# NVIDIA/spark-rapids

Measured on AMD Instinct MI355X. Metric: NDS power-run fact rows/s from on-disk parquet (speedup vs CPU backend in config), higher is better.
Workload: dtype decimal(7,2)+fp64+string-keys

## Files before the change

### native/hipdf/include/hipdf.h

```cpp
#ifndef HIPDF_H
#define HIPDF_H

#include <hip/hip_runtime.h>
#include <stddef.h>
#include <stdint.h>

#ifdef __cplusplus
#define HIPDF_STATIC_ASSERT(cond, msg) static_assert(cond, msg)
extern "C" {
#else
#define HIPDF_STATIC_ASSERT(cond, msg) _Static_assert(cond, msg)
#endif

typedef enum {
  HIPDF_U8 = 0,
  HIPDF_I8 = 1,
  HIPDF_I16 = 2,
  HIPDF_I32 = 3,
  HIPDF_I64 = 4,
  HIPDF_F32 = 5,
  HIPDF_F64 = 6,
} HipdfType;

typedef struct {
// ... 520 lines not shown
                           const void* stop, const void* bvalid,
                           const void* step, const void* svalid,
                           void* out_len, void* vout, void* err, int64_t n,
                           hipStream_t stream);
void hipdf_sequence_fill(int t, const void* offs, const void* start,
                         const void* stop, const void* step, int64_t n,
                         void* out, int64_t total, hipStream_t stream);
void hipdf_array_join_sizes(const void* offsets, const void* rvalid,
                            const void* eoffs, const void* cvalid, int dlen,
                            int rlen, int64_t n, void* contrib, int64_t total,
                            hipStream_t stream);
void hipdf_array_join_rows(const void* offsets, const void* scanned, int dlen,
                           int64_t n, void* out_len, hipStream_t stream);
void hipdf_array_join_write(const void* offsets, const void* rvalid,
                            const void* eoffs, const void* bytes,
                            const void* cvalid, const void* delim, int dlen,
                            const void* repl, int rlen, const void* scanned,
                            const void* out_off, int64_t n, void* out,
                            int64_t total, hipStream_t stream);

int64_t hipdf_pq_plain_pieces(const void* chunk, int64_t nbytes,
                              int64_t num_values, int max_def, int phys_width,
                              int64_t* out, int64_t max_out);

typedef struct {
  const void* src;
  int64_t nbytes;
  int32_t phys_width;
  int32_t dst_width;
  void* dst;
  int64_t num_values;
  int32_t group;
  int32_t max_def;
} HipdfScanChunk;
HIPDF_STATIC_ASSERT(sizeof(HipdfScanChunk) == 48, "packed as <qqiiqqii");

typedef struct HipdfScanReader HipdfScanReader;
HipdfScanReader* hipdf_scan_open(int n_threads, int n_streams,
                                 int64_t piece_bytes);
int64_t hipdf_scan_submit(HipdfScanReader* r, const HipdfScanChunk* chunks,
                          int64_t n_chunks, int n_groups,
                          hipStream_t consumer);
int hipdf_scan_wait_group(HipdfScanReader* r, int64_t ticket, int group,
                          hipStream_t consumer);
void hipdf_scan_cancel(HipdfScanReader* r, int64_t ticket);
void hipdf_scan_close(HipdfScanReader* r);

int hipdf_pool_init(double fraction, size_t bytes);
int hipdf_pool_active(void);
typedef int (*hipdf_failure_cb)(size_t needed, int retry);
void hipdf_pool_set_failure_cb(hipdf_failure_cb cb);
size_t hipdf_pool_used(void);
size_t hipdf_pool_reserved(void);
size_t hipdf_pool_high_watermark(void);
size_t hipdf_pool_overflow(void);
void* hipdf_pool_alloc(size_t n);
void hipdf_pool_free(void* p);
void* hipdf_torch_malloc(size_t size, int device, hipStream_t stream);
void hipdf_torch_free(void* ptr, size_t size, int device,
                      hipStream_t stream);
int hipdf_pool_selftest(void);

#ifdef __cplusplus
}
#endif
#undef HIPDF_STATIC_ASSERT

#endif
// ... 1 lines not shown
```

### native/hipdf/kernels/pq_pieces.h

```cpp
#ifndef HIPDF_PQ_PIECES_H
#define HIPDF_PQ_PIECES_H

#include <stdint.h>

namespace pq_pieces {

constexpr int64_t kErrTruncated = -1;
constexpr int64_t kErrDictionary = -2;
constexpr int64_t kErrEncoding = -3;
constexpr int64_t kErrCompressed = -4;
constexpr int64_t kErrWidth = -5;
constexpr int64_t kErrNulls = -6;
constexpr int64_t kErrNested = -7;
constexpr int64_t kErrMalformed = -8;
constexpr int64_t kErrCapacity = -9;
constexpr int64_t kErrCount = -10;

struct Cursor {
  const uint8_t* p;
  int64_t pos;
  int64_t end;
  bool ok;

  int byte() {
// ... 92 lines not shown
      return 0;
    }
    return last;
  }
};

inline void skip_struct(Cursor& c, int depth) {
  if (depth > 8) {
    c.ok = false;
    return;
  }
  Fields f(c);
  int t;
  while (f.next(&t)) skip_value(c, t, depth);
}

inline bool rle_all_valid(const uint8_t* lv, int64_t nb, int64_t n,
                          int max_def) {
  Cursor c{lv, 0, nb, true};
  int64_t seen = 0;
  while (seen < n) {
    uint64_t h = c.varint();
    if (!c.ok) return false;
    if (h & 1) return false;
    uint64_t count = h >> 1;
    int v = c.byte();
    if (!c.ok || v != max_def || count == 0) return false;
    if (count > (uint64_t)(n - seen)) count = (uint64_t)(n - seen);
    seen += (int64_t)count;
  }
  return true;
}

inline int64_t walk(const uint8_t* chunk, int64_t nbytes, int64_t num_values,
                    int max_def, int phys_width, int64_t* out,
                    int64_t max_out) {
  if (phys_width != 4 && phys_width != 8) return kErrWidth;
  if (nbytes < 0 || num_values < 0 || max_def < 0 || max_def > 127)
    return kErrMalformed;
  Cursor c{chunk, 0, nbytes, true};
  int64_t decoded = 0, npages = 0;
  while (decoded < num_values && c.pos < nbytes) {
    int64_t type = -1, usize = -1, csize = -1;
    int64_t n = -1, enc = -1, nulls = 0, def_len = 0, rep_len = 0;
    bool v2 = false, have_dp = false, v2_compressed = true;
    Fields f(c);
    int t;
    int fid;
    while ((fid = f.next(&t)) != 0) {
      if (fid == 1 && t == CT_I32) {
        type = c.zigzag();
      } else if (fid == 2 && t == CT_I32) {
        usize = c.zigzag();
      } else if (fid == 3 && t == CT_I32) {
        csize = c.zigzag();
      } else if (fid == 5 && t == CT_STRUCT) {
        have_dp = true;
        Fields g(c);
        int t2, f2;
        while ((f2 = g.next(&t2)) != 0) {
          if (f2 == 1 && t2 == CT_I32)
            n = c.zigzag();
          else if (f2 == 2 && t2 == CT_I32)
            enc = c.zigzag();
          else
            skip_value(c, t2, 1);
        }
      } else if (fid == 7 && t == CT_STRUCT) {
        return kErrDictionary;
      } else if (fid == 8 && t == CT_STRUCT) {
        have_dp = v2 = true;
        Fields g(c);
        int t2, f2;
        while ((f2 = g.next(&t2)) != 0) {
          if (f2 == 1 && t2 == CT_I32)
            n = c.zigzag();
          else if (f2 == 2 && t2 == CT_I32)
            nulls = c.zigzag();
          else if (f2 == 4 && t2 == CT_I32)
            enc = c.zigzag();
          else if (f2 == 5 && t2 == CT_I32)
            def_len = c.zigzag();
          else if (f2 == 6 && t2 == CT_I32)
            rep_len = c.zigzag();
          else if (f2 == 7 && (t2 == CT_TRUE || t2 == CT_FALSE))
            v2_compressed = t2 == CT_TRUE;
          else
            skip_value(c, t2, 1);
        }
      } else {
        skip_value(c, t, 0);
      }
      if (!c.ok) return kErrTruncated;
    }
    if (!c.ok) return kErrTruncated;
    if (type == 2) return kErrDictionary;
    if ((type != 0 && type != 3) || !have_dp || (type == 3) != v2)
      return kErrMalformed;
    if (usize < 0 || csize < 0 || n < 0) return kErrMalformed;
    if (csize > nbytes - c.pos) return kErrTruncated;
    if (enc != 0) return kErrEncoding;
    if (csize != usize) return kErrCompressed;
    const int64_t page = c.pos;
    int64_t vpos = 0;
    if (!v2) {
      if (max_def > 0) {
        if (csize < 4) return kErrTruncated;
        uint32_t len = (uint32_t)chunk[page] | (uint32_t)chunk[page + 1] << 8 |
                       (uint32_t)chunk[page + 2] << 16 |
                       (uint32_t)chunk[page + 3] << 24;
        if ((int64_t)len > csize - 4) return kErrTruncated;
        if (!rle_all_valid(chunk + page + 4, (int64_t)len, n, max_def))
          return kErrNulls;
        vpos = 4 + (int64_t)len;
      }
    } else {
      if (rep_len != 0) return kErrNested;
      if (def_len < 0 || def_len > csize) return kErrMalformed;
      if (max_def > 0) {
        if (nulls != 0) return kErrNulls;
        if (!rle_all_valid(chunk + page, def_len, n, max_def))
          return kErrNulls;
      } else if (def_len != 0) {
        return kErrMalformed;
      }
      (void)v2_compressed;
      vpos = def_len;
    }
    if (csize - vpos != n * (int64_t)phys_width) return kErrCompressed;
    if (n > num_values - decoded) return kErrCount;
    if (npages >= max_out) return kErrCapacity;
    out[3 * npages] = page + vpos;
    out[3 * npages + 1] = n * (int64_t)phys_width;
    out[3 * npages + 2] = n;
    ++npages;
    decoded += n;
    c.pos = page + csize;
  }
  if (decoded != num_values) return decoded < num_values ? kErrTruncated
                                                         : kErrCount;
  return npages;
}

}

#endif
```

### native/hipdf/scan_reader.hip

```cpp
#include <hip/hip_runtime.h>

#include <algorithm>
#include <condition_variable>
#include <deque>
#include <memory>
#include <mutex>
#include <thread>
#include <vector>

#include "hipdf.h"
#include "pq_pieces.h"

namespace {

__global__ void k_widen_i32_i64(const int32_t* __restrict__ in,
                                int64_t* __restrict__ out, int64_t n) {
  int64_t i = (int64_t)blockIdx.x * blockDim.x + threadIdx.x;
  int64_t stride = (int64_t)gridDim.x * blockDim.x;
  for (; i < n; i += stride) out[i] = (int64_t)in[i];
}

struct Piece {
  const uint8_t* src;
  uint8_t* dst;
  int64_t nbytes;
  int32_t widen;
  int32_t group;
};

struct Group {
  int64_t total = 0;
  int64_t enqueued = 0;
  int open_workers = 0;
  std::vector<hipEvent_t> events;
  bool waited = false;
};

struct Submit {
  int64_t ticket = 0;
  std::vector<Piece> pieces;
  size_t next = 0;
  std::vector<Group> groups;
  hipEvent_t start = nullptr;
  int in_flight = 0;
  bool cancelled = false;
  int error = 0;
  std::vector<char> stream_used;

  bool group_ready(int g) const {
    const Group& gr = groups[(size_t)g];
    return gr.enqueued == gr.total && gr.open_workers == 0;
  }
  bool exhausted() const { return cancelled || next >= pieces.size(); }
};

}

struct HipdfScanReader {
  int device = 0;
  int64_t piece_bytes = 0;
  std::vector<std::thread> threads;
  std::vector<hipStream_t> streams;
  std::vector<hipStream_t> owned_streams;
  std::vector<void*> scratch;
  std::mutex mu;
  std::condition_variable work_cv;
  std::condition_variable done_cv;
  std::deque<std::shared_ptr<Submit>> queue;
  std::vector<std::shared_ptr<Submit>> live;
  int64_t next_ticket = 1;
  bool stop = false;

  std::shared_ptr<Submit> find(int64_t ticket) {
    for (auto& s : live)
      if (s->ticket == ticket) return s;
    return nullptr;
  }

  void leave_group(Submit& s, int g, int w) {
    hipEvent_t ev = nullptr;
    hipError_t e = hipEventCreateWithFlags(&ev, hipEventDisableTiming);
    if (e == hipSuccess) e = hipEventRecord(ev, streams[(size_t)w]);
    std::lock_guard<std::mutex> lk(mu);
    if (e != hipSuccess && !s.error) s.error = (int)e;
    if (ev) s.groups[(size_t)g].events.push_back(ev);
    --s.groups[(size_t)g].open_workers;
    done_cv.notify_all();
  }

  void worker(int w) {
    (void)hipSetDevice(device);
    std::shared_ptr<Submit> cur;
    int cur_group = -1;
    for (;;) {
      std::shared_ptr<Submit> s;
      size_t idx = 0;
      {
        std::unique_lock<std::mutex> lk(mu);
        for (;;) {
          while (!queue.empty() && queue.front()->exhausted())
            queue.pop_front();
          if (stop || !queue.empty()) break;
          if (cur) break;
          work_cv.wait(lk);
        }
        if (!stop && !queue.empty()) {
          s = queue.front();
          idx = s->next++;
          int g = s->pieces[idx].group;
          if (s != cur || g != cur_group) ++s->groups[(size_t)g].open_workers;
          ++s->in_flight;
        }
      }
      if (cur && (!s || s != cur || s->pieces[idx].group != cur_group)) {
        leave_group(*cur, cur_group, w);
        cur.reset();
        cur_group = -1;
      }
      if (!s) {
        std::lock_guard<std::mutex> lk(mu);
        if (stop) return;
        continue;
      }
      const Piece& p = s->pieces[idx];
      hipStream_t st = streams[(size_t)w];
      hipError_t e = hipSuccess;
      if (!s->stream_used[(size_t)w]) {
        e = hipStreamWaitEvent(st, s->start, 0);
        s->stream_used[(size_t)w] = 1;
      }
      if (e == hipSuccess) {
        if (!p.widen) {
          e = hipMemcpyAsync(p.dst, p.src, (size_t)p.nbytes,
                             hipMemcpyHostToDevice, st);
        } else {
          e = hipMemcpyAsync(scratch[(size_t)w], p.src, (size_t)p.nbytes,
                             hipMemcpyHostToDevice, st);
          if (e == hipSuccess) {
            int64_t n = p.nbytes / 4;
            int blocks = (int)std::min<int64_t>((n + 255) / 256, 4096);
            hipLaunchKernelGGL(k_widen_i32_i64, dim3((unsigned)blocks),
                               dim3(256), 0, st,
                               (const int32_t*)scratch[(size_t)w],
                               (int64_t*)p.dst, n);
            e = hipGetLastError();
          }
        }
      }
      cur = s;
      cur_group = p.group;
      {
        std::lock_guard<std::mutex> lk(mu);
        if (e != hipSuccess && !s->error) s->error = (int)e;
        ++s->groups[(size_t)p.group].enqueued;
        --s->in_flight;
        done_cv.notify_all();
      }
    }
  }
};

extern "C" {

int64_t hipdf_pq_plain_pieces(const void* chunk, int64_t nbytes,
                              int64_t num_values, int max_def, int phys_width,
                              int64_t* out, int64_t max_out) {
  return pq_pieces::walk((const uint8_t*)chunk, nbytes, num_values, max_def,
                         phys_width, out, max_out);
}

HipdfScanReader* hipdf_scan_open(int n_threads, int n_streams,
                                 int64_t piece_bytes) {
  n_threads = std::max(1, std::min(n_threads, 8));
  n_streams = std::max(1, std::min(n_streams, n_threads));
  piece_bytes = std::max<int64_t>(piece_bytes, 64) / 8 * 8;
  auto* r = new HipdfScanReader();
  r->piece_bytes = piece_bytes;
  if (hipGetDevice(&r->device) != hipSuccess) {
    delete r;
    return nullptr;
  }
  bool ok = true;
  for (int i = 0; i < n_streams && ok; ++i) {
    hipStream_t st = nullptr;
    ok = hipStreamCreateWithFlags(&st, hipStreamNonBlocking) == hipSuccess;
    if (ok) r->owned_streams.push_back(st);
  }
  for (int w = 0; w < n_threads && ok; ++w) {
    void* p = nullptr;
    ok = hipMalloc(&p, (size_t)piece_bytes) == hipSuccess;
    if (ok) r->scratch.push_back(p);
  }
  if (!ok) {
    for (void* p : r->scratch) (void)hipFree(p);
    for (hipStream_t st : r->owned_streams) (void)hipStreamDestroy(st);
    delete r;
    return nullptr;
  }
  for (int w = 0; w < n_threads; ++w)
    r->streams.push_back(r->owned_streams[(size_t)(w % n_streams)]);
  for (int w = 0; w < n_threads; ++w)
    r->threads.emplace_back([r, w] { r->worker(w); });
  return r;
}

int64_t hipdf_scan_submit(HipdfScanReader* r, const HipdfScanChunk* chunks,
                          int64_t n_chunks, int n_groups,
                          hipStream_t consumer) {
  if (!r || n_chunks < 0 || n_groups < 0) return -100;
  auto s = std::make_shared<Submit>();
  s->groups.resize((size_t)n_groups);
  s->stream_used.assign(r->threads.size(), 0);
  std::vector<int64_t> pages;
  for (int64_t i = 0; i < n_chunks; ++i) {
    const HipdfScanChunk& c = chunks[i];
    if (c.group < 0 || c.group >= n_groups) return -100;
    bool widen = c.phys_width == 4 && c.dst_width == 8;
    if (!widen && c.dst_width != c.phys_width) return pq_pieces::kErrWidth;
    if (pages.empty()) pages.resize(3 * 256);
    int64_t np;
    for (;;) {
      np = pq_pieces::walk((const uint8_t*)c.src, c.nbytes, c.num_values,
                           c.max_def, c.phys_width, pages.data(),
                           (int64_t)pages.size() / 3);
      if (np != pq_pieces::kErrCapacity || pages.size() >= (3u << 22)) break;
      pages.resize(pages.size() * 4);
    }
    if (np < 0) return np;
    int64_t row = 0;
    for (int64_t k = 0; k < np; ++k) {
      int64_t off = pages[(size_t)(3 * k)], nb = pages[(size_t)(3 * k + 1)];
      for (int64_t done = 0; done < nb; done += r->piece_bytes) {
        int64_t take = std::min(r->piece_bytes, nb - done);
        Piece p;
        p.src = (const uint8_t*)c.src + off + done;
        p.dst = (uint8_t*)c.dst +
                (row + done / c.phys_width) * (int64_t)c.dst_width;
        p.nbytes = take;
        p.widen = widen ? 1 : 0;
        p.group = c.group;
        s->pieces.push_back(p);
      }
      row += pages[(size_t)(3 * k + 2)];
    }
  }
  std::stable_sort(s->pieces.begin(), s->pieces.end(),
                   [](const Piece& a, const Piece& b) {
                     return a.group < b.group;
                   });
  for (const Piece& p : s->pieces) ++s->groups[(size_t)p.group].total;
  if (hipEventCreateWithFlags(&s->start, hipEventDisableTiming) != hipSuccess)
    return -101;
  if (hipEventRecord(s->start, consumer) != hipSuccess) {
// ... 23 lines not shown
  for (hipEvent_t ev : g.events)
    if (hipStreamWaitEvent(consumer, ev, 0) != hipSuccess) return -102;
  g.waited = true;
  return 0;
}

void hipdf_scan_cancel(HipdfScanReader* r, int64_t ticket) {
  if (!r) return;
  std::shared_ptr<Submit> s;
  bool drain = false;
  {
    std::unique_lock<std::mutex> lk(r->mu);
    s = r->find(ticket);
    if (!s) return;
    s->cancelled = true;
    r->work_cv.notify_all();
    r->done_cv.notify_all();
    r->done_cv.wait(lk, [&] {
      if (s->in_flight) return false;
      for (const Group& g : s->groups)
        if (g.open_workers) return false;
      return true;
    });
    for (const Group& g : s->groups)
      if (!g.waited && g.enqueued) drain = true;
    r->live.erase(std::find(r->live.begin(), r->live.end(), s));
  }
  if (drain)
    for (size_t w = 0; w < s->stream_used.size(); ++w)
      if (s->stream_used[w]) (void)hipStreamSynchronize(r->streams[w]);
  for (Group& g : s->groups)
    for (hipEvent_t ev : g.events) (void)hipEventDestroy(ev);
  (void)hipEventDestroy(s->start);
}

void hipdf_scan_close(HipdfScanReader* r) {
  if (!r) return;
  std::vector<int64_t> tickets;
  {
    std::lock_guard<std::mutex> lk(r->mu);
    for (auto& s : r->live) tickets.push_back(s->ticket);
  }
  for (int64_t t : tickets) hipdf_scan_cancel(r, t);
  {
    std::lock_guard<std::mutex> lk(r->mu);
    r->stop = true;
    r->work_cv.notify_all();
    r->done_cv.notify_all();
  }
  for (std::thread& t : r->threads) t.join();
  for (hipStream_t st : r->owned_streams) {
    (void)hipStreamSynchronize(st);
    (void)hipStreamDestroy(st);
  }
  for (void* p : r->scratch) (void)hipFree(p);
  delete r;
}

}
```

### spark_rapids_amd/api.py

```python
from __future__ import annotations

from typing import Dict, Iterable, List, Optional, Sequence, Union

import numpy as np

from .column import Column, ColumnBatch, Field, Schema
from .config import RapidsConf, CONCURRENT_GPU_TASKS
from .expr.aggregates import AggExpr
from .expr.expressions import Expression, col as _col
from .memory.semaphore import GpuSemaphore
from .plan import logical as L
from .plan.overrides import plan_physical
from .types import DType, INT32, TypeId


class MemTable:

    def __init__(self, batches: List[ColumnBatch], schema: Schema,
                 replicated: bool = False):
        self.batches = batches
        self.schema = schema
        self.replicated = replicated

    def partitions(self) -> Iterable[ColumnBatch]:
# ... 449 lines not shown
                    pending, nbytes = [], 0
                pending.append(b)
                nbytes += b.nbytes
            if pending:
                merged.append(pending[0] if len(pending) == 1
                              else _ops.concat_batches(pending))
            batches = merged
        return DataFrame(self, L.Scan(MemTable(batches, schema, replicated),
                                      schema, label))

    def register(self, name: str, df: DataFrame):
        self.catalog[name] = df

    def table(self, name: str) -> DataFrame:
        return self.catalog[name]

    def sql(self, query: str) -> DataFrame:
        from .sql.parser import parse_sql

        return parse_sql(self, query)

    def read_parquet(self, path: str, columns=None,
                     replicated: bool = False) -> DataFrame:
        import torch

        from .config import PARQUET_MT_THREADS, PARQUET_READER_TYPE
        from .io.parquet import ParquetTable

        reader = str(self.conf.get(PARQUET_READER_TYPE)).upper()
        if reader == "AUTO":
            reader = "GPU_DECODE" if (torch.cuda.is_available()
                                      and self.conf.sql_enabled) else "CPU"
        from .config import (BATCH_SIZE_BYTES, PARQUET_STREAM_SCAN,
                             PARQUET_STREAM_SCAN_FILES)

        src = ParquetTable(path, columns=columns, reader=reader,
                           prefetch_threads=self.conf.get(PARQUET_MT_THREADS),
                           replicated=replicated,
                           chunk_bytes=self.conf.get(BATCH_SIZE_BYTES),
                           stream_scan=self.conf.get(PARQUET_STREAM_SCAN),
                           stream_files=self.conf.get(
                               PARQUET_STREAM_SCAN_FILES))
        return DataFrame(self, L.Scan(src, src.schema, f"parquet:{path}"))

    def write_parquet(self, df: DataFrame, path: str,
                      compression: str = "snappy",
                      gpu_encode: bool = False):
        if gpu_encode:
            from . import ops as _ops
            from .io.parquet_write import write_parquet_gpu

            exec_ = df.physical_plan()
            sem = GpuSemaphore.get()
            with sem.held():
                root = exec_
                while type(root).__name__ == "DeviceTransferExec":
                    root = root.children[0]
                batches = list(root.execute())
                if not batches:
                    batches = [ColumnBatch(
                        [Column.from_pylist([], f.dtype).cuda()
                         for f in df.schema.fields], 0)]
                batch = batches[0] if len(batches) == 1 \
                    else _ops.concat_batches(batches)
                write_parquet_gpu(batch, df.schema, path)
            return
        from .io.parquet import write_parquet

        batch = df.collect_batch()
        write_parquet(batch, df.schema, path, compression)

    def range(self, start: int, end: Optional[int] = None,
              step: int = 1, num_partitions: int = 1) -> DataFrame:
        if end is None:
            start, end = 0, start
# ... 125 lines not shown
```

### spark_rapids_amd/config.py

```python
from __future__ import annotations

import threading
from dataclasses import dataclass
from typing import Any, Callable, Dict, Optional


@dataclass
class ConfEntry:
    key: str
    default: Any
    doc: str
    conv: Callable[[str], Any]
    startup_only: bool = False
    internal: bool = False


_REGISTRY: Dict[str, ConfEntry] = {}


def _register(entry: ConfEntry) -> ConfEntry:
    assert entry.key not in _REGISTRY, f"duplicate conf key {entry.key}"
    _REGISTRY[entry.key] = entry
    return entry

# ... 106 lines not shown
OPTIMIZER_EXPLAIN = bool_conf(
    "spark.rapids.sql.optimizer.explain", False,
    "Print the cost-based optimizer's estimates for every plan.")
SHUFFLE_WAVE_BYTES = bytes_conf(
    "spark.rapids.shuffle.wave.bytes", 1 << 30,
    "Bytes budget per exchange wave: a shuffle whose serialized send "
    "buffers exceed this is split into multiple all-to-all rounds so the "
    "exchange memory stays bounded (bounce-buffer windowing analogue).")
PINNED_POOL_SIZE = bytes_conf(
    "spark.rapids.memory.pinnedPool.size", 8 << 30,
    "Size of the pinned host memory pool used for spill and H2D/D2H staging.")
HOST_SPILL_STORAGE_SIZE = bytes_conf(
    "spark.rapids.memory.host.spillStorageSize", 32 << 30,
    "Maximum bytes of host memory used to hold spilled device buffers before "
    "spilling further to disk.")
SPILL_PATH = str_conf(
    "spark.rapids.memory.spillPath", "/tmp/rapids_spill",
    "Local directory for disk spill files.")
PARQUET_READER_TYPE = str_conf(
    "spark.rapids.sql.format.parquet.reader.type", "AUTO",
    "Parquet reader: AUTO (GPU decode when a GPU is present, CPU otherwise), "
    "GPU_DECODE (hipdf kernels decode PLAIN/dictionary pages on device, "
    "per-file CPU fallback for unsupported features), CPU (pyarrow host "
    "decode feeding device batches — the hybrid-scan analogue).")
PARQUET_ENABLED = bool_conf(
    "spark.rapids.sql.format.parquet.enabled", True,
    "Enable parquet scans on GPU.")
PARQUET_MT_THREADS = int_conf(
    "spark.rapids.sql.format.parquet.multiThreadedRead.numThreads", 8,
    "Threads in the multithreaded parquet prefetch pool.")
PARQUET_STREAM_SCAN = bool_conf(
    "spark.rapids.sql.format.parquet.streamScan.enabled", True,
    "A multi-file GPU_DECODE scan whose selected column chunks are all "
    "uncompressed PLAIN fixed-width pages without nulls is uploaded by the "
    "native in-order reader: the files arrive one after the other straight "
    "in their destination columns, the scan yields one batch per group of "
    "files while the later files are still being copied, and the upload "
    "starts when the query starts. Any other scan runs as before.")
PARQUET_STREAM_SCAN_FILES = int_conf(
    "spark.rapids.sql.format.parquet.streamScan.filesPerBatch", 4,
    "Files per batch of a stream scan. Fewer files per batch let more of "
    "the query's kernels run while later files are still being copied, and "
    "launch every per-batch kernel more often; measured on MI355X with 8 "
    "fact files, 4 was the best of 1, 2 and 4.")
BROADCAST_THRESHOLD = bytes_conf(
    "spark.rapids.sql.join.broadcastThreshold", 512 << 20,
    "Distributed joins all-gather (broadcast) the build side when its "
    "global size is below this; larger builds hash-exchange BOTH sides "
    "across ranks instead (shuffled hash join).")
SHUFFLE_MODE = str_conf(
    "spark.rapids.shuffle.mode", "MULTITHREADED",
    "Shuffle transport: MULTITHREADED (host staging) or RCCL (device-to-device "
    "all-to-all over xGMI).")
SHUFFLE_PARTITIONS = int_conf(
    "spark.rapids.sql.shuffle.partitions", 16,
    "Default number of shuffle partitions per GPU for exchanges.")
SHUFFLE_COMPRESS = str_conf(
    "spark.rapids.shuffle.compression.codec", "none",
    "Codec for host-path shuffle payloads (none|zstd|lz4|snappy). Device "
    "(RCCL/xGMI) shuffles stay uncompressed: the links outrun a host "
    "compression round-trip.")
RETRY_MAX_SPLITS = int_conf(
    "spark.rapids.sql.retry.maxSplits", 8,
    "Maximum recursive batch splits attempted by the OOM retry framework "
    "before giving up.")
GPU_OOM_INJECTION = int_conf(
    "spark.rapids.sql.test.injectOOM", 0, "Inject a synthetic GPU OOM on the "
    "Nth tracked allocation (testing only, 0 = off).", internal=True)
STABLE_SORT = bool_conf(
    "spark.rapids.sql.stableSort.enabled", False,
    "Use a stable sort on GPU (matches CPU tie ordering; slightly slower).")
PRUNE_COLUMNS = bool_conf(
    "spark.rapids.sql.optimizer.pruneColumns.enabled", True,
    "Push projections below joins/aggregates so unused columns are never "
    "gathered or transferred (Catalyst-optimizer analogue).")
JOIN_SUBPARTITION_BYTES = int_conf(
    "spark.rapids.sql.join.subPartition.targetBytes", 1 << 30,
# ... 111 lines not shown
```

### spark_rapids_amd/io/parquet.py

```python
from __future__ import annotations

import concurrent.futures as cf
import glob
import os
from typing import Iterable, List, Optional

import numpy as np
import torch

from ..column import Column, ColumnBatch, Field, Schema
from ..types import (BOOL, DATE32, DType, FLOAT32, FLOAT64, INT8, INT16,
                     INT32, INT64, STRING, TIMESTAMP, TypeId)

_PA_TYPES = None


def _pa():
    import pyarrow

    return pyarrow


def arrow_to_dtype(t) -> DType:
    import pyarrow as pa
# ... 135 lines not shown
    md, _, _ = _file_meta(path)
    if md.num_row_groups == 0:
        return set()
    name_to_idx = {md.row_group(0).column(j).path_in_schema: j
                   for j in range(md.num_columns)}
    keep = set()
    for rg in range(md.num_row_groups):
        rgmd = md.row_group(rg)
        ok = True
        for name, op, value in triples:
            j = name_to_idx.get(name)
            if j is None:
                continue
            st = rgmd.column(j).statistics
            if st is None or not st.has_min_max:
                continue
            if not _stat_overlaps(op, value, st.min, st.max):
                ok = False
                break
        if ok:
            keep.add(rg)
            SCAN_STATS["rg_scanned"] += 1
        else:
            SCAN_STATS["rg_skipped"] += 1
    return keep


class ParquetTable:

    def __init__(self, path: str, num_partitions: int = 0,
                 columns: Optional[List[str]] = None, reader: str = "CPU",
                 prefetch_threads: int = 4, replicated: bool = False,
                 chunk_bytes: int = 0, stream_scan: bool = False,
                 stream_files: int = 4, stream_piece_bytes: int = 0):
        self.stream_scan = stream_scan
        self.stream_files = stream_files
        self.stream_piece_bytes = stream_piece_bytes
        self.chunk_bytes = chunk_bytes
        self.replicated = replicated
        if isinstance(path, (list, tuple)):
            self.files = list(path)
        else:
            self.files = sorted(glob.glob(path)) \
                if any(ch in path for ch in "*?") \
                else ([os.path.join(path, f) for f in sorted(os.listdir(path))
                       if f.endswith(".parquet")]
                      if os.path.isdir(path) else [path])
        if not self.files:
            raise FileNotFoundError(path)
        self.columns = columns
        self.reader = reader
        self.prefetch_threads = prefetch_threads
        self.schema = parquet_schema(self.files[0])
        if columns:
            keep = [f for f in self.schema.fields if f.name in columns]
            self.schema = Schema(keep)

    def _clone(self) -> "ParquetTable":
        t = ParquetTable.__new__(ParquetTable)
        t.replicated = self.replicated
        t.files = self.files
        t.columns = self.columns
        t.reader = self.reader
        t.prefetch_threads = self.prefetch_threads
        t.schema = self.schema
        t.rg_predicate = getattr(self, "rg_predicate", None)
        t.chunk_bytes = getattr(self, "chunk_bytes", 0)
        t.stream_scan = getattr(self, "stream_scan", False)
        t.stream_files = getattr(self, "stream_files", 4)
        t.stream_piece_bytes = getattr(self, "stream_piece_bytes", 0)
        return t

    def with_columns(self, names: List[str]) -> "ParquetTable":
        t = self._clone()
        t.columns = list(names)
        t.schema = Schema([f for f in self.schema.fields if f.name in names])
        return t

    def with_predicate(self, triples) -> "ParquetTable":
        t = self._clone()
        t.rg_predicate = list(triples)
        return t

    def _read_one(self, path: str) -> List[ColumnBatch]:
        from .filecache import get_cached, put_cached

        cached = get_cached(path, self.columns)
        if cached is not None:
            return cached if isinstance(cached, list) else [cached]
        batches = self._read_one_uncached(path)
        put_cached(path, self.columns, batches)
        return batches

    def _rg_chunks(self, path: str, keep):
        budget = getattr(self, "chunk_bytes", 0)
        if not budget:
            return None
        from .parquet_gpu import _file_meta

        md, _, _ = _file_meta(path)
        rgs = [r for r in range(md.num_row_groups)
               if keep is None or r in keep]
        if len(rgs) <= 1:
# ... 228 lines not shown
```

### spark_rapids_amd/io/parquet_gpu.py

```python
from __future__ import annotations

import struct as pystruct
from typing import List, Optional

import numpy as np
import torch

from ..column import Column, ColumnBatch, mask_nbytes
from ..types import DType, TypeId
from . import thrift_compact as tc

PLAIN, PLAIN_DICTIONARY, RLE, RLE_DICTIONARY = 0, 2, 3, 8
DELTA_BINARY_PACKED = 5
DELTA_LENGTH_BYTE_ARRAY, DELTA_BYTE_ARRAY = 6, 7
DATA_PAGE, DICTIONARY_PAGE, DATA_PAGE_V2 = 0, 2, 3

_PHYS_NP = {
    "INT32": np.dtype("<i4"),
    "INT64": np.dtype("<i8"),
    "FLOAT": np.dtype("<f4"),
    "DOUBLE": np.dtype("<f8"),
}


# ... 899 lines not shown
                return None
            fdt = [arrow_to_dtype(arrow_schema.field(n).type)
                   for n in columns]
            if dtypes is None:
                dtypes = fdt
            elif [d.id for d in fdt] != [d.id for d in dtypes]:
                return None
            name_to_idx = {md.row_group(0).column(j).path_in_schema: j
                           for j in range(md.num_columns)} \
                if md.num_row_groups else {}
            chunks = []
            rows = 0
            for rg in range(md.num_row_groups):
                if keep is not None and rg not in keep:
                    continue
                rgmd = md.row_group(rg)
                for ci, (name, dt) in enumerate(zip(columns, fdt)):
                    j = name_to_idx.get(name)
                    if j is None or dt.is_nested \
                            or dt.id in (TypeId.STRING, TypeId.BOOL):
                        return None
                    sc = pq_schema.column(j)
                    cmd = rgmd.column(j)
                    pw = _PHYS_WIDTH.get(cmd.physical_type)
                    dw = torch.empty(0, dtype=torch_dtype(dt)).element_size()
                    if pw is None or sc.max_repetition_level > 0 \
                            or cmd.compression != "UNCOMPRESSED" \
                            or cmd.has_dictionary_page \
                            or not (dw == pw or (cmd.physical_type == "INT32"
                                                 and dw == 8
                                                 and dt.is_decimal)) \
                            or cmd.num_values != rgmd.num_rows:
                        return None
                    chunks.append((ci, cmd.data_page_offset,
                                   cmd.total_compressed_size, pw, dw,
                                   cmd.num_values, sc.max_definition_level,
                                   rows))
                rows += rgmd.num_rows
            per_file.append((rows, chunks))
        if dtypes is None:
            return None
        return dtypes, per_file

    layout = build()
    if len(_STREAM_LAYOUTS) > 256:
        _STREAM_LAYOUTS.clear()
    _STREAM_LAYOUTS[key] = (mtimes, layout)
    return layout


class StreamScan:

    def __init__(self, reader: int, ticket: int, batches, keepalive):
        self._reader = reader
        self._ticket = ticket
        self._batches = batches
        self._keepalive = keepalive

    @staticmethod
    def start(table, files) -> Optional["StreamScan"]:
        from ..column import torch_dtype
        from ..ops.gpu_backend import _stream, ext
        from .parquet import PHASE_STATS

        layout = _stream_layout(table, files)
        if layout is None:
            return None
        dtypes, per_file = layout
        per_batch = max(1, int(getattr(table, "stream_files", 1)))
        tdts = [torch_dtype(d) for d in dtypes]
        batches = []
        descs = []
        keepalive = []
        nbytes = 0
        for g in range(0, len(files), per_batch):
            group = per_file[g:g + per_batch]
            rows = sum(r for r, _ in group)
            bufs = [torch.empty(max(rows, 1), dtype=t, device="cuda")[:rows]
                    for t in tdts]
            base = 0
            for path, (frows, chunks) in zip(files[g:g + per_batch], group):
                mm = _file_mmap(path)
                keepalive.append(mm)
                for ci, off, nb, pw, dw, nvals, max_def, row0 in chunks:
                    if off < 0 or off + nb > mm[3]:
                        return None
                    descs.append((mm[2] + off, nb, pw, dw,
                                  bufs[ci].data_ptr() + (base + row0) * dw,
                                  nvals, len(batches), max_def))
                    nbytes += nvals * pw
                base += frows
            batches.append(ColumnBatch(
                [Column(d, rows, b, None, null_count=0)
                 for d, b in zip(dtypes, bufs)], rows))
        table_np = np.array(descs, dtype=np.dtype(
            [("src", "<i8"), ("nbytes", "<i8"), ("pw", "<i4"), ("dw", "<i4"),
             ("dst", "<i8"), ("n", "<i8"), ("group", "<i4"),
             ("max_def", "<i4")]))
        reader = _reader(table.prefetch_threads,
                         getattr(table, "stream_piece_bytes", 0)
                         or STREAM_PIECE_BYTES)
        ticket = ext.scan_submit(reader, table_np.ctypes.data, len(descs),
                                 len(batches), _stream())
        if ticket <= 0:
            if ticket <= -100:
                raise RuntimeError(f"hipdf scan_submit failed rc={ticket}")
            return None
        PHASE_STATS["upload_bytes"] += nbytes
        return StreamScan(reader, ticket, batches, keepalive)

    def batches(self):
        from ..ops.gpu_backend import _stream, ext

        try:
            for g in range(len(self._batches)):
                rc = ext.scan_wait_group(self._reader, self._ticket, g,
                                         _stream())
                if rc != 0:
                    raise RuntimeError(f"stream scan failed rc={rc}")
                batch, self._batches[g] = self._batches[g], None
                yield batch
        finally:
            self.close()

    def close(self):
        from ..ops.gpu_backend import ext

        if self._ticket:
            ticket, self._ticket = self._ticket, 0
            ext.scan_cancel(self._reader, ticket)
            self._batches = []
# ... 2 lines not shown
```

Before: 2.311 billion.

## Stream nullable PLAIN columns through native scan reader with host-decoded validity

Extends the native in-order parquet stream reader to accept nullable columns with max definition level 1. Worker threads decode each page's RLE/bit-packed definition levels into a host bitmask with per-tile popcount prefixes, upload the dense values, mask and tile table per slice, and a kernel scatters values to their rows while writing the validity bitmap. Scans over NDS fact tables whose columns contain nulls previously fell back to the slower file-by-file path; now they can use the overlapped streaming upload. The cost is host-side level decoding, extra small copies per slice and a scatter kernel launch per slice.

```diff
diff --git a/native/hipdf/include/hipdf.h b/native/hipdf/include/hipdf.h
--- a/native/hipdf/include/hipdf.h
+++ b/native/hipdf/include/hipdf.h
@@ -576,8 +576,10 @@
   int64_t num_values;
   int32_t group;
   int32_t max_def;
+  void* valid;
+  int64_t valid_bit0;
 } HipdfScanChunk;
-HIPDF_STATIC_ASSERT(sizeof(HipdfScanChunk) == 48, "packed as <qqiiqqii");
+HIPDF_STATIC_ASSERT(sizeof(HipdfScanChunk) == 64, "packed as <qqiiqqiiqq");
 
 typedef struct HipdfScanReader HipdfScanReader;
 HipdfScanReader* hipdf_scan_open(int n_threads, int n_streams,
diff --git a/native/hipdf/kernels/pq_levels.h b/native/hipdf/kernels/pq_levels.h
--- /dev/null
+++ b/native/hipdf/kernels/pq_levels.h
@@ -0,0 +1,107 @@
+#ifndef HIPDF_PQ_LEVELS_H
+#define HIPDF_PQ_LEVELS_H
+
+#include <stdint.h>
+#include <string.h>
+
+#include "pq_pieces.h"
+
+namespace pq_pieces {
+
+constexpr int64_t kErrLevels = -11;
+
+constexpr int kLevelStride = 5;
+constexpr int kTileRows = 2048;
+
+inline int64_t walk_levels(const uint8_t* chunk, int64_t nbytes,
+                           int64_t num_values, int max_def, int phys_width,
+                           int64_t* out, int64_t max_out) {
+  return walk_impl(chunk, nbytes, num_values, max_def, phys_width, out,
+                   max_out, true);
+}
+
+inline int64_t mask_bytes(int64_t n) {
+  return (n + kTileRows - 1) / kTileRows * (kTileRows / 8);
+}
+inline int64_t tile_entries(int64_t n) {
+  return (n + kTileRows - 1) / kTileRows + 1;
+}
+
+inline void fill_ones(uint8_t* mask, int64_t pos, int64_t count) {
+  int64_t end = pos + count;
+  int64_t b0 = pos >> 3, b1 = end >> 3;
+  if (b0 == b1) {
+    mask[b0] |= (uint8_t)(((1u << count) - 1u) << (pos & 7));
+    return;
+  }
+  if (pos & 7) {
+    mask[b0] |= (uint8_t)(0xFFu << (pos & 7));
+    ++b0;
+  }
+  if (b1 > b0) memset(mask + b0, 0xFF, (size_t)(b1 - b0));
+  if (end & 7) mask[b1] |= (uint8_t)((1u << (end & 7)) - 1u);
+}
+
+inline int64_t decode_levels(const uint8_t* lv, int64_t nb, int64_t n,
+                             uint8_t* mask, uint32_t* tiles) {
+  if (nb < 0 || n < 0 || n > INT32_MAX) return kErrMalformed;
+  memset(mask, 0, (size_t)mask_bytes(n));
+  Cursor c{lv, 0, nb, true};
+  int64_t pos = 0;
+  while (pos < n) {
+    uint64_t h = c.varint();
+    if (!c.ok) return kErrTruncated;
+    uint64_t count = h >> 1;
+    if (count == 0) return kErrLevels;
+    if (!(h & 1)) {
+      int v = c.byte();
+      if (!c.ok) return kErrTruncated;
+      if (v != 0 && v != 1) return kErrLevels;
+      if (count > (uint64_t)(n - pos)) count = (uint64_t)(n - pos);
+      if (v) fill_ones(mask, pos, (int64_t)count);
+      pos += (int64_t)count;
+      continue;
+    }
+    uint64_t rows = count > (uint64_t)(n - pos + 7) / 8
+                        ? (uint64_t)(n - pos)
+                        : count * 8;
+    if (rows > (uint64_t)(n - pos)) rows = (uint64_t)(n - pos);
+    const int64_t bytes = (int64_t)((rows + 7) / 8);
+    const int64_t at = c.pos;
+    c.advance((uint64_t)bytes);
+    if (!c.ok) return kErrTruncated;
+    const uint8_t* src = lv + at;
+    const int sh = (int)(pos & 7);
+    uint8_t* dst = mask + (pos >> 3);
+    const int tail = (int)(rows & 7);
+    if (sh == 0) {
+      memcpy(dst, src, (size_t)bytes);
+      if (tail) dst[bytes - 1] &= (uint8_t)((1u << tail) - 1u);
+    } else {
+      for (int64_t i = 0; i < bytes; ++i) {
+        unsigned b = src[i];
+        if (tail && i == bytes - 1) b &= (1u << tail) - 1u;
+        dst[i] |= (uint8_t)(b << sh);
+        if (b >> (8 - sh)) dst[i + 1] |= (uint8_t)(b >> (8 - sh));
+      }
+    }
+    pos += (int64_t)rows;
+  }
+  const int64_t ntiles = tile_entries(n) - 1;
+  uint32_t total = 0;
+  for (int64_t t = 0; t < ntiles; ++t) {
+    tiles[t] = total;
+    const uint8_t* p = mask + t * (kTileRows / 8);
+    for (int w = 0; w < kTileRows / 64; ++w) {
+      uint64_t word;
+      memcpy(&word, p + 8 * w, 8);
+      total += (uint32_t)__builtin_popcountll(word);
+    }
+  }
+  tiles[ntiles] = total;
+  return (int64_t)total;
+}
+
+}
+
+#endif
diff --git a/native/hipdf/kernels/pq_pieces.h b/native/hipdf/kernels/pq_pieces.h
--- a/native/hipdf/kernels/pq_pieces.h
+++ b/native/hipdf/kernels/pq_pieces.h
@@ -148,12 +148,14 @@
   return true;
 }
 
-inline int64_t walk(const uint8_t* chunk, int64_t nbytes, int64_t num_values,
-                    int max_def, int phys_width, int64_t* out,
-                    int64_t max_out) {
+inline int64_t walk_impl(const uint8_t* chunk, int64_t nbytes,
+                         int64_t num_values, int max_def, int phys_width,
+                         int64_t* out, int64_t max_out, bool with_levels) {
+  const int stride = with_levels ? 5 : 3;
   if (phys_width != 4 && phys_width != 8) return kErrWidth;
   if (nbytes < 0 || num_values < 0 || max_def < 0 || max_def > 127)
     return kErrMalformed;
+  if (with_levels && max_def > 1) return kErrNulls;
   Cursor c{chunk, 0, nbytes, true};
   int64_t decoded = 0, npages = 0;
   while (decoded < num_values && c.pos < nbytes) {
@@ -219,6 +221,7 @@
     if (csize != usize) return kErrCompressed;
     const int64_t page = c.pos;
     int64_t vpos = 0;
+    int64_t lpos = 0, llen = 0;
     if (!v2) {
       if (max_def > 0) {
         if (csize < 4) return kErrTruncated;
@@ -226,29 +229,45 @@
                        (uint32_t)chunk[page + 2] << 16 |
                        (uint32_t)chunk[page + 3] << 24;
         if ((int64_t)len > csize - 4) return kErrTruncated;
-        if (!rle_all_valid(chunk + page + 4, (int64_t)len, n, max_def))
+        if (!with_levels &&
+            !rle_all_valid(chunk + page + 4, (int64_t)len, n, max_def))
           return kErrNulls;
+        lpos = 4;
+        llen = (int64_t)len;
         vpos = 4 + (int64_t)len;
       }
     } else {
       if (rep_len != 0) return kErrNested;
       if (def_len < 0 || def_len > csize) return kErrMalformed;
       if (max_def > 0) {
-        if (nulls != 0) return kErrNulls;
-        if (!rle_all_valid(chunk + page, def_len, n, max_def))
-          return kErrNulls;
+        if (!with_levels) {
+          if (nulls != 0) return kErrNulls;
+          if (!rle_all_valid(chunk + page, def_len, n, max_def))
+            return kErrNulls;
+        }
+        llen = def_len;
       } else if (def_len != 0) {
         return kErrMalformed;
       }
       (void)v2_compressed;
       vpos = def_len;
     }
-    if (csize - vpos != n * (int64_t)phys_width) return kErrCompressed;
+    const int64_t vbytes = csize - vpos;
+    if (with_levels && max_def > 0) {
+      if (vbytes % phys_width != 0 || vbytes > n * (int64_t)phys_width)
+        return kErrCompressed;
+    } else if (vbytes != n * (int64_t)phys_width) {
+      return kErrCompressed;
+    }
     if (n > num_values - decoded) return kErrCount;
     if (npages >= max_out) return kErrCapacity;
-    out[3 * npages] = page + vpos;
-    out[3 * npages + 1] = n * (int64_t)phys_width;
-    out[3 * npages + 2] = n;
+    out[stride * npages] = page + vpos;
+    out[stride * npages + 1] = vbytes;
+    out[stride * npages + 2] = n;
+    if (with_levels) {
+      out[stride * npages + 3] = page + lpos;
+      out[stride * npages + 4] = llen;
+    }
     ++npages;
     decoded += n;
     c.pos = page + csize;
@@ -258,6 +277,13 @@
   return npages;
 }
 
+inline int64_t walk(const uint8_t* chunk, int64_t nbytes, int64_t num_values,
+                    int max_def, int phys_width, int64_t* out,
+                    int64_t max_out) {
+  return walk_impl(chunk, nbytes, num_values, max_def, phys_width, out,
+                   max_out, false);
+}
+
 }
 
 #endif
diff --git a/native/hipdf/scan_reader.hip b/native/hipdf/scan_reader.hip
--- a/native/hipdf/scan_reader.hip
+++ b/native/hipdf/scan_reader.hip
@@ -9,15 +9,60 @@
 #include <vector>
 
 #include "hipdf.h"
+#include "pq_levels.h"
 #include "pq_pieces.h"
 
 namespace {
+
+constexpr int kTile = pq_pieces::kTileRows;
 
 __global__ void k_widen_i32_i64(const int32_t* __restrict__ in,
                                 int64_t* __restrict__ out, int64_t n) {
   int64_t i = (int64_t)blockIdx.x * blockDim.x + threadIdx.x;
   int64_t stride = (int64_t)gridDim.x * blockDim.x;
   for (; i < n; i += stride) out[i] = (int64_t)in[i];
+}
+
+template <typename SrcT, typename DstT>
+__global__ void k_place_nullable(const SrcT* __restrict__ src,
+                                 const uint64_t* __restrict__ mask,
+                                 const uint32_t* __restrict__ tiles,
+                                 DstT* __restrict__ dst,
+                                 uint32_t* __restrict__ valid, int64_t bit0,
+                                 int64_t n) {
+  const int64_t d = (bit0 & ~(int64_t)63) + (int64_t)blockIdx.x * blockDim.x +
+                    threadIdx.x;
+  const int64_t r = d - bit0;
+  const bool in = r >= 0 && r < n;
+  bool v = false;
+  if (in) {
+    const int64_t wi = r >> 6;
+    const uint64_t word = mask[wi];
+    v = (word >> (r & 63)) & 1;
+    DstT out = (DstT)0;
+    if (v) {
+      const int64_t tile = r / kTile;
+      uint32_t rank = tiles[tile] - tiles[0];
+      for (int64_t w = tile * (kTile / 64); w < wi; ++w)
+        rank += (uint32_t)__popcll(mask[w]);
+      rank += (uint32_t)__popcll(word & (((uint64_t)1 << (r & 63)) - 1));
+      out = (DstT)src[rank];
+    }
+    dst[r] = out;
+  }
+  const uint64_t bits = __ballot(v);
+  const uint64_t rows = __ballot(in);
+  if ((threadIdx.x & 63) == 0 && rows) {
+    uint32_t* w32 = valid + (d >> 6) * 2;
+    const uint32_t lo = (uint32_t)bits, hi = (uint32_t)(bits >> 32);
+    if (rows == ~(uint64_t)0) {
+      w32[0] = lo;
+      w32[1] = hi;
+    } else {
+      if (lo) atomicOr(&w32[0], lo);
+      if (hi) atomicOr(&w32[1], hi);
+    }
+  }
 }
 
 struct Piece {
@@ -26,6 +71,13 @@
   int64_t nbytes;
   int32_t widen;
   int32_t group;
+  uint32_t* valid = nullptr;
+  int64_t bit0 = 0;
+  int64_t rows = 0;
+  const uint8_t* levels = nullptr;
+  int64_t level_bytes = 0;
+  int32_t phys_width = 0;
+  uint8_t* host = nullptr;
 };
 
 struct Group {
@@ -52,6 +104,13 @@
     return gr.enqueued == gr.total && gr.open_workers == 0;
   }
   bool exhausted() const { return cancelled || next >= pieces.size(); }
+  void release_host() {
+    for (Piece& p : pieces) {
+      delete[] p.host;
+      p.host = nullptr;
+    }
+  }
+  ~Submit() { release_host(); }
 };
 
 }
@@ -63,6 +122,9 @@
   std::vector<hipStream_t> streams;
   std::vector<hipStream_t> owned_streams;
   std::vector<void*> scratch;
+  int64_t value_cap = 0;
+  int64_t mask_cap = 0;
+  int64_t tiles_cap = 0;
   std::mutex mu;
   std::condition_variable work_cv;
   std::condition_variable done_cv;
@@ -86,6 +148,68 @@
     if (ev) s.groups[(size_t)g].events.push_back(ev);
     --s.groups[(size_t)g].open_workers;
     done_cv.notify_all();
+  }
+
+  int64_t slice_rows(int width) const {
+    return std::max<int64_t>(kTile, piece_bytes / width / kTile * kTile);
+  }
+
+  int nullable_piece(Piece& p, int w, hipStream_t st) {
+    using namespace pq_pieces;
+    const int64_t n = p.rows;
+    if (n == 0) return p.nbytes == 0 ? 0 : (int)kErrCount;
+    const int64_t mb = mask_bytes(n), te = tile_entries(n);
+    p.host = new (std::nothrow) uint8_t[(size_t)(mb + te * 4)];
+    if (!p.host) return (int)hipErrorOutOfMemory;
+    uint32_t* tiles = (uint32_t*)(p.host + mb);
+    int64_t nvalid = decode_levels(p.levels, p.level_bytes, n, p.host, tiles);
+    if (nvalid < 0) return (int)nvalid;
+    if (nvalid * p.phys_width != p.nbytes) return (int)kErrCount;
+    uint8_t* vals = (uint8_t*)scratch[(size_t)w];
+    uint8_t* dmask = vals + value_cap;
+    uint8_t* dtiles = dmask + mask_cap;
+    const int dst_width = p.widen ? 8 : p.phys_width;
+    const int64_t step = slice_rows(p.phys_width);
+    for (int64_t r0 = 0; r0 < n; r0 += step) {
+      const int64_t rows = std::min(step, n - r0);
+      const int64_t t0 = r0 / kTile, t1 = t0 + (rows + kTile - 1) / kTile;
+      const int64_t v0 = tiles[t0], v1 = tiles[t1];
+      hipError_t e = hipSuccess;
+      if (v1 > v0)
+        e = hipMemcpyAsync(vals, p.src + v0 * p.phys_width,
+                           (size_t)((v1 - v0) * p.phys_width),
+                           hipMemcpyHostToDevice, st);
+      if (e == hipSuccess)
+        e = hipMemcpyAsync(dmask, p.host + t0 * (kTile / 8),
+                           (size_t)((rows + 63) / 64 * 8),
+                           hipMemcpyHostToDevice, st);
+      if (e == hipSuccess)
+        e = hipMemcpyAsync(dtiles, tiles + t0, (size_t)((t1 - t0 + 1) * 4),
+                           hipMemcpyHostToDevice, st);
+      if (e != hipSuccess) return (int)e;
+      const int64_t bit0 = p.bit0 + r0;
+      const int64_t span = (bit0 & 63) + rows;
+      dim3 grid((unsigned)((span + 255) / 256)), block(256);
+      uint8_t* dst = p.dst + r0 * dst_width;
+      if (p.widen)
+        hipLaunchKernelGGL((k_place_nullable<int32_t, int64_t>), grid, block,
+                           0, st, (const int32_t*)vals,
+                           (const uint64_t*)dmask, (const uint32_t*)dtiles,
+                           (int64_t*)dst, p.valid, bit0, rows);
+      else if (p.phys_width == 4)
+        hipLaunchKernelGGL((k_place_nullable<uint32_t, uint32_t>), grid,
+                           block, 0, st, (const uint32_t*)vals,
+                           (const uint64_t*)dmask, (const uint32_t*)dtiles,
+                           (uint32_t*)dst, p.valid, bit0, rows);
+      else
+        hipLaunchKernelGGL((k_place_nullable<uint64_t, uint64_t>), grid,
+                           block, 0, st, (const uint64_t*)vals,
+                           (const uint64_t*)dmask, (const uint32_t*)dtiles,
+                           (uint64_t*)dst, p.valid, bit0, rows);
+      e = hipGetLastError();
+      if (e != hipSuccess) return (int)e;
+    }
+    return 0;
   }
 
   void worker(int w) {
@@ -122,15 +246,17 @@
         if (stop) return;
         continue;
       }
-      const Piece& p = s->pieces[idx];
+      Piece& p = s->pieces[idx];
       hipStream_t st = streams[(size_t)w];
-      hipError_t e = hipSuccess;
+      int e = hipSuccess;
       if (!s->stream_used[(size_t)w]) {
         e = hipStreamWaitEvent(st, s->start, 0);
         s->stream_used[(size_t)w] = 1;
       }
       if (e == hipSuccess) {
-        if (!p.widen) {
+        if (p.valid) {
+          e = nullable_piece(p, w, st);
+        } else if (!p.widen) {
           e = hipMemcpyAsync(p.dst, p.src, (size_t)p.nbytes,
                              hipMemcpyHostToDevice, st);
         } else {
@@ -151,7 +277,7 @@
       cur_group = p.group;
       {
         std::lock_guard<std::mutex> lk(mu);
-        if (e != hipSuccess && !s->error) s->error = (int)e;
+        if (e != hipSuccess && !s->error) s->error = e;
         ++s->groups[(size_t)p.group].enqueued;
         --s->in_flight;
         done_cv.notify_all();
@@ -176,6 +302,9 @@
   piece_bytes = std::max<int64_t>(piece_bytes, 64) / 8 * 8;
   auto* r = new HipdfScanReader();
   r->piece_bytes = piece_bytes;
+  r->value_cap = std::max<int64_t>(piece_bytes, kTile * 8);
+  r->mask_cap = r->slice_rows(4) / 8;
+  r->tiles_cap = (r->slice_rows(4) / kTile + 1) * 4;
   if (hipGetDevice(&r->device) != hipSuccess) {
     delete r;
     return nullptr;
@@ -188,7 +317,8 @@
   }
   for (int w = 0; w < n_threads && ok; ++w) {
     void* p = nullptr;
-    ok = hipMalloc(&p, (size_t)piece_bytes) == hipSuccess;
+    ok = hipMalloc(&p, (size_t)(r->value_cap + r->mask_cap +
+                                r->tiles_cap)) == hipSuccess;
     if (ok) r->scratch.push_back(p);
   }
   if (!ok) {
@@ -219,6 +349,38 @@
     if (!widen && c.dst_width != c.phys_width) return pq_pieces::kErrWidth;
     if (pages.empty()) pages.resize(3 * 256);
     int64_t np;
+    if (c.valid) {
+      if (c.max_def != 1 || c.valid_bit0 < 0) return -100;
+      const int ls = pq_pieces::kLevelStride;
+      for (;;) {
+        np = pq_pieces::walk_levels((const uint8_t*)c.src, c.nbytes,
+                                    c.num_values, c.max_def, c.phys_width,
+                                    pages.data(), (int64_t)pages.size() / ls);
+        if (np != pq_pieces::kErrCapacity || pages.size() >= (3u << 22))
+          break;
+        pages.resize(pages.size() * 4);
+      }
+      if (np < 0) return np;
+      int64_t row = 0;
+      for (int64_t k = 0; k < np; ++k) {
+        const int64_t* pg = &pages[(size_t)(ls * k)];
+        Piece p;
+        p.src = (const uint8_t*)c.src + pg[0];
+        p.dst = (uint8_t*)c.dst + row * (int64_t)c.dst_width;
+        p.nbytes = pg[1];
+        p.widen = widen ? 1 : 0;
+        p.group = c.group;
+        p.valid = (uint32_t*)c.valid;
+        p.bit0 = c.valid_bit0 + row;
+        p.rows = pg[2];
+        p.levels = (const uint8_t*)c.src + pg[3];
+        p.level_bytes = pg[4];
+        p.phys_width = c.phys_width;
+        s->pieces.push_back(p);
+        row += pg[2];
+      }
+      continue;
+    }
     for (;;) {
       np = pq_pieces::walk((const uint8_t*)c.src, c.nbytes, c.num_values,
                            c.max_def, c.phys_width, pages.data(),
@@ -308,6 +470,7 @@
   for (Group& g : s->groups)
     for (hipEvent_t ev : g.events) (void)hipEventDestroy(ev);
   (void)hipEventDestroy(s->start);
+  s->release_host();
 }
 
 void hipdf_scan_close(HipdfScanReader* r) {
diff --git a/spark_rapids_amd/api.py b/spark_rapids_amd/api.py
--- a/spark_rapids_amd/api.py
+++ b/spark_rapids_amd/api.py
@@ -505,7 +505,8 @@
             reader = "GPU_DECODE" if (torch.cuda.is_available()
                                       and self.conf.sql_enabled) else "CPU"
         from .config import (BATCH_SIZE_BYTES, PARQUET_STREAM_SCAN,
-                             PARQUET_STREAM_SCAN_FILES)
+                             PARQUET_STREAM_SCAN_FILES,
+                             PARQUET_STREAM_SCAN_NULLS)
 
         src = ParquetTable(path, columns=columns, reader=reader,
                            prefetch_threads=self.conf.get(PARQUET_MT_THREADS),
@@ -513,7 +514,9 @@
                            chunk_bytes=self.conf.get(BATCH_SIZE_BYTES),
                            stream_scan=self.conf.get(PARQUET_STREAM_SCAN),
                            stream_files=self.conf.get(
-                               PARQUET_STREAM_SCAN_FILES))
+                               PARQUET_STREAM_SCAN_FILES),
+                           stream_nulls=self.conf.get(
+                               PARQUET_STREAM_SCAN_NULLS))
         return DataFrame(self, L.Scan(src, src.schema, f"parquet:{path}"))
 
     def write_parquet(self, df: DataFrame, path: str,
diff --git a/spark_rapids_amd/config.py b/spark_rapids_amd/config.py
--- a/spark_rapids_amd/config.py
+++ b/spark_rapids_amd/config.py
@@ -162,7 +162,8 @@
 PARQUET_STREAM_SCAN = bool_conf(
     "spark.rapids.sql.format.parquet.streamScan.enabled", True,
     "A multi-file GPU_DECODE scan whose selected column chunks are all "
-    "uncompressed PLAIN fixed-width pages without nulls is uploaded by the "
+    "uncompressed PLAIN fixed-width pages (with nulls: see "
+    "streamScan.nulls.enabled) is uploaded by the "
     "native in-order reader: the files arrive one after the other straight "
     "in their destination columns, the scan yields one batch per group of "
     "files while the later files are still being copied, and the upload "
@@ -173,6 +174,13 @@
     "the query's kernels run while later files are still being copied, and "
     "launch every per-batch kernel more often; measured on MI355X with 8 "
     "fact files, 4 was the best of 1, 2 and 4.")
+PARQUET_STREAM_SCAN_NULLS = bool_conf(
+    "spark.rapids.sql.format.parquet.streamScan.nulls.enabled", True,
+    "A stream scan also takes nullable columns (max definition level 1) "
+    "whose footers report nulls: the reader's worker threads decode each "
+    "page's definition levels into a validity bitmask on the host, and one "
+    "kernel per slice of a page places the dense values at their rows. "
+    "When false, a scan with such a column runs file by file as before.")
 BROADCAST_THRESHOLD = bytes_conf(
     "spark.rapids.sql.join.broadcastThreshold", 512 << 20,
     "Distributed joins all-gather (broadcast) the build side when its "
diff --git a/spark_rapids_amd/io/parquet.py b/spark_rapids_amd/io/parquet.py
--- a/spark_rapids_amd/io/parquet.py
+++ b/spark_rapids_amd/io/parquet.py
@@ -191,8 +191,10 @@
                  columns: Optional[List[str]] = None, reader: str = "CPU",
                  prefetch_threads: int = 4, replicated: bool = False,
                  chunk_bytes: int = 0, stream_scan: bool = False,
-                 stream_files: int = 4, stream_piece_bytes: int = 0):
+                 stream_files: int = 4, stream_piece_bytes: int = 0,
+                 stream_nulls: bool = False):
         self.stream_scan = stream_scan
+        self.stream_nulls = stream_nulls
         self.stream_files = stream_files
         self.stream_piece_bytes = stream_piece_bytes
         self.chunk_bytes = chunk_bytes
@@ -228,6 +230,7 @@
         t.stream_scan = getattr(self, "stream_scan", False)
         t.stream_files = getattr(self, "stream_files", 4)
         t.stream_piece_bytes = getattr(self, "stream_piece_bytes", 0)
+        t.stream_nulls = getattr(self, "stream_nulls", False)
         return t
 
     def with_columns(self, names: List[str]) -> "ParquetTable":
diff --git a/spark_rapids_amd/io/parquet_gpu.py b/spark_rapids_amd/io/parquet_gpu.py
--- a/spark_rapids_amd/io/parquet_gpu.py
+++ b/spark_rapids_amd/io/parquet_gpu.py
@@ -955,10 +955,15 @@
                                                  and dt.is_decimal)) \
                             or cmd.num_values != rgmd.num_rows:
                         return None
+                    st = cmd.statistics if cmd.is_stats_set else None
+                    nulls = st.null_count \
+                        if st is not None and st.has_null_count else None
+                    if cmd.num_values == 0:
+                        nulls = 0
                     chunks.append((ci, cmd.data_page_offset,
                                    cmd.total_compressed_size, pw, dw,
                                    cmd.num_values, sc.max_definition_level,
-                                   rows))
+                                   rows, nulls))
                 rows += rgmd.num_rows
             per_file.append((rows, chunks))
         if dtypes is None:
@@ -991,6 +996,7 @@
             return None
         dtypes, per_file = layout
         per_batch = max(1, int(getattr(table, "stream_files", 1)))
+        take_nulls = bool(getattr(table, "stream_nulls", False))
         tdts = [torch_dtype(d) for d in dtypes]
         batches = []
         descs = []
@@ -1001,25 +1007,47 @@
             rows = sum(r for r, _ in group)
             bufs = [torch.empty(max(rows, 1), dtype=t, device="cuda")[:rows]
                     for t in tdts]
+            masks = [None] * len(tdts)
+            null_counts = [0] * len(tdts)
+            for _, chunks in group:
+                for ch in chunks:
+                    ci, max_def, nulls = ch[0], ch[6], ch[8]
+                    if max_def == 0 or nulls == 0:
+                        continue
+                    if max_def != 1 or not take_nulls:
+                        return None
+                    if masks[ci] is None:
+                        masks[ci] = torch.zeros(mask_nbytes(rows),
+                                                dtype=torch.uint8,
+                                                device="cuda")
+                    null_counts[ci] = None if nulls is None \
+                        or null_counts[ci] is None else null_counts[ci] + nulls
             base = 0
             for path, (frows, chunks) in zip(files[g:g + per_batch], group):
                 mm = _file_mmap(path)
                 keepalive.append(mm)
-                for ci, off, nb, pw, dw, nvals, max_def, row0 in chunks:
+                for ci, off, nb, pw, dw, nvals, max_def, row0, _ in chunks:
                     if off < 0 or off + nb > mm[3]:
+                        return None
+                    m = masks[ci]
+                    if m is not None and max_def != 1:
                         return None
                     descs.append((mm[2] + off, nb, pw, dw,
                                   bufs[ci].data_ptr() + (base + row0) * dw,
-                                  nvals, len(batches), max_def))
-                    nbytes += nvals * pw
+                                  nvals, len(batches), max_def,
+                                  m.data_ptr() if m is not None else 0,
+                                  base + row0))
+                    nbytes += nvals * pw if m is None else nb
                 base += frows
             batches.append(ColumnBatch(
-                [Column(d, rows, b, None, null_count=0)
-                 for d, b in zip(dtypes, bufs)], rows))
+                [Column(d, rows, b, m, null_count=0 if m is None else nc)
+                 for d, b, m, nc in zip(dtypes, bufs, masks, null_counts)],
+                rows))
         table_np = np.array(descs, dtype=np.dtype(
             [("src", "<i8"), ("nbytes", "<i8"), ("pw", "<i4"), ("dw", "<i4"),
              ("dst", "<i8"), ("n", "<i8"), ("group", "<i4"),
-             ("max_def", "<i4")]))
+             ("max_def", "<i4"), ("valid", "<i8"),
+             ("valid_bit0", "<i8")]))
         reader = _reader(table.prefetch_threads,
                          getattr(table, "stream_piece_bytes", 0)
                          or STREAM_PIECE_BYTES)
```

After: 2.614 billion (median of 6 runs). +13.1%, better.
